# vandenheuvel/rust-lp

Hardware: AMD Instinct MI355X
Metric: simplex iterations/sec (higher is better)
Workload: dtype f64; 1 GPU; dense10k: synthetic dense LP 10000x10000 f64 (+10000 slack columns), SteepestDescent, dense tableau with blocked f64-MFMA updates; m=10000, n=10000, seed=20250002, engine=tableau, update_block=64, parallelism=single GPU, solves=1

## Files before the change

include/relp_engine.h:

```cpp
#ifndef RELP_ENGINE_H
#define RELP_ENGINE_H

#include <stdint.h>

#ifdef __cplusplus
extern "C" {
#endif

typedef struct relp_engine relp_engine_t;

typedef enum {
    RELP_OK = 0,
    RELP_E_ARG = -1,
    RELP_E_HIP = -2,
    RELP_E_ZERO_PIVOT = -3,
    RELP_E_SINGULAR = -4,
    RELP_E_STATE = -5,
    RELP_E_UNSUPPORTED = -6,
    RELP_E_ALLOC = -7
} relp_status_t;

typedef enum {
    RELP_RUNNING = 0,
    RELP_OPTIMAL = 1,
// ... 134 lines not shown
                                  const double *rhs, relp_cutpool_t **pool);
relp_status_t relp_cutpool_destroy(relp_engine_t *h, relp_cutpool_t *pool);
relp_status_t relp_cutpool_set_active(relp_engine_t *h, relp_cutpool_t *pool, const int32_t *ids, int32_t count, int32_t flag);
relp_status_t relp_cutpool_slacks(relp_engine_t *h, relp_cutpool_t *pool, double *out_count);
relp_status_t relp_cutpool_separate(relp_engine_t *h, relp_cutpool_t *pool, int32_t segments, double tol, int32_t by_efficacy,
                                    int32_t *ids_out , double *slack_out , int32_t *found);
relp_status_t relp_cutpool_add(relp_engine_t *h, relp_cutpool_t *pool, const int32_t *ids, int32_t count);
relp_status_t relp_cutpool_stats(const relp_engine_t *h, const relp_cutpool_t *pool, int64_t *out4);
relp_status_t relp_from_basis(relp_engine_t *h, const int32_t *basis_columns_m);
relp_status_t relp_set_reinversion_interval(relp_engine_t *h, int64_t pivots);
int64_t       relp_reinversions(const relp_engine_t *h);
relp_status_t relp_flush(relp_engine_t *h);
relp_status_t relp_tab_flush_stats(relp_engine_t *h, int64_t *out2);
relp_status_t relp_retab_stats(const relp_engine_t *h, int64_t *out4);
int32_t       relp_tab_load_batch(const relp_engine_t *h);
int32_t       relp_update_block(const relp_engine_t *h);
relp_status_t relp_lu_stats(const relp_engine_t *h, int64_t *out8);
relp_status_t relp_lu_lookahead_stats(const relp_engine_t *h, int64_t *out4);
relp_status_t relp_lu_kernel_layout(const relp_engine_t *h, int32_t *out4);
relp_status_t relp_lu_set_device_factorisation(relp_engine_t *h, int32_t on);
relp_status_t relp_lu_device_factorisation_stats(const relp_engine_t *h, int64_t *out6);
relp_status_t relp_lu_factor_residual(relp_engine_t *h, double *out);

relp_status_t relp_lu_phase_cycles(relp_engine_t *h, int64_t *out16);

relp_status_t relp_basis_inverse_row(relp_engine_t *h, int32_t row, double *out_m);
relp_status_t relp_should_refactor(relp_engine_t *h, int32_t *out);
relp_status_t relp_generate_column_of(relp_engine_t *h, const int32_t *row_idx, const double *values, int32_t nnz, double *out_m);
relp_status_t relp_cost_difference_of(relp_engine_t *h, const int32_t *row_idx, const double *values, int32_t nnz, double *out);
relp_status_t relp_lu_change_basis(relp_engine_t *h, int32_t pivot_row_index);
// ... 71 lines not shown
```

rust-lp_amd/csrc/relp_abi.cpp:

```cpp
#include <cstring>
#include <new>

#include "relp_engine.hpp"

using relp::Engine;

struct relp_engine { Engine impl; };

#define H(h) ((h)->impl)

extern "C" {

void relp_default_config(relp_config_t* cfg) {
    std::memset(cfg, 0, sizeof(*cfg));
    cfg->device = -1;
    cfg->phase_one_rule = RELP_RULE_FIRST_PROFITABLE_WITH_MEMORY;
    cfg->phase_two_rule = RELP_RULE_STEEPEST_DESCENT;
    cfg->tol_cost = 1e-7; cfg->tol_pivot = 1e-5; cfg->tol_zero = 1e-11; cfg->tol_tie = 1e-9; cfg->tol_feas = 1e-7;
    cfg->poll_interval = 64;
    cfg->trace_capacity = 0;
    cfg->shard_rank = 0; cfg->shard_count = 1;
    cfg->update_block = -1;
    cfg->engine = RELP_ENGINE_REVISED;
}
// ... 132 lines not shown
                                    double* slack_out, int32_t* found) {
    return h ? H(h).cutpool_separate(pool, segments, tol, by_efficacy, ids_out, slack_out, found) : RELP_E_ARG;
}
relp_status_t relp_cutpool_add(relp_engine_t* h, relp_cutpool_t* pool, const int32_t* ids, int32_t count) { return h ? H(h).cutpool_add(pool, ids, count) : RELP_E_ARG; }
relp_status_t relp_cutpool_stats(const relp_engine_t* h, const relp_cutpool_t* pool, int64_t* out4) { return (h && out4) ? H(h).cutpool_stats(pool, out4) : RELP_E_ARG; }
relp_status_t relp_solve_relaxation(relp_engine_t* h, int64_t max_iters, int32_t* outcome) {
    return h ? H(h).solve_relaxation(max_iters, outcome) : RELP_E_ARG;
}
relp_status_t relp_from_basis(relp_engine_t* h, const int32_t* basis) { return (h && basis) ? H(h).from_basis(basis) : RELP_E_ARG; }

relp_status_t relp_flush(relp_engine_t* h) { return h ? H(h).flush() : RELP_E_ARG; }
relp_status_t relp_set_reinversion_interval(relp_engine_t* h, int64_t pivots) { return h ? H(h).set_reinversion_interval(pivots) : RELP_E_ARG; }
int64_t relp_reinversions(const relp_engine_t* h) { return h ? H(h).reinversions() : -1; }
int32_t relp_update_block(const relp_engine_t* h) { return h ? H(h).update_block() : -1; }
int32_t relp_tab_load_batch(const relp_engine_t* h) { return h ? H(h).tab_load_batch_size() : -1; }
relp_status_t relp_lu_stats(const relp_engine_t* h, int64_t* out8) { return (h && out8) ? H(h).lu_stats(out8) : RELP_E_ARG; }
relp_status_t relp_lu_lookahead_stats(const relp_engine_t* h, int64_t* out4) { return (h && out4) ? H(h).lu_lookahead_stats(out4) : RELP_E_ARG; }
relp_status_t relp_lu_kernel_layout(const relp_engine_t* h, int32_t* out4) { return (h && out4) ? H(h).lu_kernel_layout(out4) : RELP_E_ARG; }
relp_status_t relp_lu_set_device_factorisation(relp_engine_t* h, int32_t on) { return h ? H(h).lu_set_device_factorisation(on != 0) : RELP_E_ARG; }
relp_status_t relp_lu_factor_residual(relp_engine_t* h, double* out) { return (h && out) ? H(h).lu_factor_residual(out) : RELP_E_ARG; }
relp_status_t relp_lu_device_factorisation_stats(const relp_engine_t* h, int64_t* out6) { return (h && out6) ? H(h).luf_stats(out6) : RELP_E_ARG; }
relp_status_t relp_shard_inject_failure(relp_engine_t* h, int64_t after_pivots) { if (!h) return RELP_E_ARG; H(h).shard_inject_failure(after_pivots); return RELP_OK; }
relp_status_t relp_lu_phase_cycles(relp_engine_t* h, int64_t* out16) { return (h && out16) ? H(h).lu_phase_cycles(out16) : RELP_E_ARG; }
relp_status_t relp_basis_inverse_row(relp_engine_t* h, int32_t row, double* out_m) { return (h && out_m) ? H(h).basis_inverse_row(row, out_m) : RELP_E_ARG; }
relp_status_t relp_should_refactor(relp_engine_t* h, int32_t* out) { return (h && out) ? H(h).should_refactor(out) : RELP_E_ARG; }
relp_status_t relp_generate_column_of(relp_engine_t* h, const int32_t* idx, const double* val, int32_t nnz, double* out_m) {
    return h ? H(h).generate_column_of(idx, val, nnz, out_m) : RELP_E_ARG;
}
relp_status_t relp_cost_difference_of(relp_engine_t* h, const int32_t* idx, const double* val, int32_t nnz, double* out) {
    return h ? H(h).cost_difference_of(idx, val, nnz, out) : RELP_E_ARG;
// ... 101 lines not shown
```

rust-lp_amd/csrc/relp_engine.cpp:

```cpp
#include "relp_engine_internal.hpp"
#include "relp_gomory.hpp"

#include <algorithm>
#include <chrono>
#include <cmath>
#include <cstdio>
#include <cstdlib>
#include <cstring>
#include <limits>

namespace relp {

bool Engine::hip_ok(hipError_t e, const char* what) {
    if (e == hipSuccess) return true;
    err_ = std::string(what) + ": " + hipGetErrorString(e);
    return false;
}

Engine::~Engine() { rccl_release(); luf_release(); }

ColumnTable Engine::table() const {
    ColumnTable ct;
    ct.nr_artificial = lay_.nr_artificial;
    ct.nr_normal = lay_.nr_normal;
// ... 55 lines not shown
    stream_ = s;
    owns_stream_ = false;
    return RELP_OK;
}

Switches Switches::read() {
    Switches s;
    auto given = [](const char* name) { return std::getenv(name) != nullptr; };
    auto num = [](const char* name, int unset) { const char* e = std::getenv(name); return e ? std::atoi(e) : unset; };
    s.debug = given("RELP_DEBUG");
    s.pivot_guard_set = given("RELP_PIVOT_GUARD");
    if (s.pivot_guard_set) s.pivot_guard = std::atof(std::getenv("RELP_PIVOT_GUARD"));
    s.tab_flush_all = num("RELP_TAB_FLUSH_ALL", 0) != 0;
    s.tab_load_batch = num("RELP_TAB_LOAD_BATCH", 0);
    s.tab_w_split = num("RELP_TAB_W_SPLIT", 0);
    s.fused_update = num("RELP_FUSED_UPDATE", 1) != 0;
    s.lu_lookahead_set = given("RELP_LU_LOOKAHEAD");
    s.lu_lookahead = num("RELP_LU_LOOKAHEAD", 8);
    s.fuse_lanes = num("RELP_FUSE_LANES", 256);
    s.lu_device_factor = num("RELP_LU_DEVICE_FACTOR", 0);
    s.lu_pipeline_short = num("RELP_LU_PIPELINE_SHORT", 0) != 0;
    s.ft_big = num("RELP_FT_BIG", -1);
    s.ft_hyper_set = given("RELP_FT_HYPER");
    s.ft_hyper = num("RELP_FT_HYPER", 0x9);
    s.ft_grid_price = given("RELP_FT_GRID_PRICE") ? (num("RELP_FT_GRID_PRICE", 0) != 0 ? 1 : 0) : -1;
    if (given("RELP_LUF_BUMP_CAP")) s.luf_bump_cap = std::max(16, num("RELP_LUF_BUMP_CAP", 0));
    s.luf_dense = std::max(0, std::min(64, num("RELP_LUF_DENSE", 64)));
    s.luf_lds = num("RELP_LUF_LDS", 1) != 0;
    s.lu_peel_stacks = num("RELP_LU_PEEL_STACKS", 0) != 0;
    s.dump_basis_set = given("RELP_DUMP_BASIS");
// ... 115 lines not shown
        HIP_TRY(dT0_.alloc(ld_t_ * n_owned));
        HIP_TRY(dR0_.alloc(ld_r_ * (block_ + 1)));
        {
            flush_all_ = sw_.tab_flush_all;
            HIP_TRY(d_fstats_.alloc(2));
            if (!flush_all_) {
                HIP_TRY(d_fcols_.alloc(n_owned));
                HIP_TRY(d_fcount_.alloc(1));
                HIP_TRY(d_fmask_.alloc((n_owned + 63) / 64));
                HIP_TRY(d_R0c_.alloc(ld_r_ * block_));
            }
        }
        {
            load_batch_ = tab_load_batch(sw_.tab_load_batch);
            w_split_ = sw_.tab_w_split >= 1 ? std::min(sw_.tab_w_split, 16) : kTabSplitDefault;
        }
        {
            fused_update_ = sw_.fused_update;
            if (cfg_.pivot_rescue && cfg_.shard_count == 1) fused_update_ = false;
            if (fused_update_) {
                HIP_TRY(d_b_alt_.alloc(ld_b_));
                HIP_TRY(d_basis_alt_.alloc(lay_.m));
                HIP_TRY(d_shadow_.alloc(std::max(block_, 1) + 1));
                HIP_TRY(d_shadow_meta_.alloc_raw(2 * sizeof(int32_t)));
                const int32_t none[2] = {-1, 0};
                HIP_TRY(d_shadow_meta_.upload(none, 2, stream_));
            }
        }
        HIP_TRY(d_cost_store_.alloc(n_store_));
        HIP_TRY(d_idcol_.alloc(lay_.m));
// ... 113 lines not shown

void Engine::enqueue_price(int cost_mode, const double* vec, const PivotRecord* rec, int32_t p_lo, int32_t p_hi) {
    const ColumnTable ct = table();
    if (lu_) {
        launch_price_csc(csc(), ct, vec, d_d_, 0, lay_.nr_normal, cost_mode, SelectPartials{}, rec, stream_);
        launch_price_virtual(ct, vec, d_d_, cost_mode, rec, stream_);
        return;
    }
    launch_price_structural(A_base(), ld_a_, ct, vec, d_d_, p_lo, p_hi, cost_mode, rec, stream_);
    if (p_lo > 0 || p_hi < lay_.nr_normal) launch_price_mask_unowned(ct, d_d_, p_lo, p_hi, rec, stream_);
    launch_price_virtual(ct, vec, d_d_, cost_mode, rec, stream_);
}

void Engine::enqueue_iteration_tableau(int rule) {
    const TableauView tv = tview();
    const DeferredUpdate du = deferred();
    const SelectPartials sp = tab_partials(rule);
    if (fused_update_ && in_loop_) {
        prof_begin(RELP_K_FTRAN);
        launch_tab_select_column_rmin(tv, du, sp, tab_scan_blocks(lay_.sc_hi - lay_.sc_lo), d_alpha_, d_b_, tolerances(), d_rmin_,
                                      d_rec_, stream_, d_shadow_, d_shadow_meta_);
        prof_end();
        prof_begin(RELP_K_PRICE);
        launch_tab_ratio_update_all(tv, du, sp, lay_.m, d_alpha_, d_b_, d_b_alt_, d_basis_, d_basis_alt_, d_in_basis_, d_trace_,
                                    trace_cap_, tolerances(), d_rmin_, d_shadow_, d_shadow_meta_, d_rec_, stream_);
        prof_end();
        d_b_.swap(d_b_alt_);
        d_basis_.swap(d_basis_alt_);
        shadow_pending_ = true;
        if (++since_flush_ >= block_) enqueue_flush();
        return;
    }
    tab_settle();
// ... 1878 lines not shown
```

rust-lp_amd/csrc/relp_engine.hpp:

```cpp
#pragma once
#include <hip/hip_runtime.h>

#include <cstdint>
#include <chrono>
#include <condition_variable>
#include <functional>
#include <memory>
#include <mutex>
#include <string>
#include <thread>
#include <vector>

#include "../../include/relp_engine.h"
#include "relp_buffers.hpp"
#include "relp_kernels.h"
#include "relp_layout.hpp"
#include "relp_cutpool.hpp"
#include "relp_lu.hpp"
#include "relp_pack.hpp"

namespace relp {
struct DevicePool {
    PoolImage image;
    DeviceBuf<int64_t> d_slice_ptr;
// ... 41 lines not shown
    ~HostPool() {
        for (Slot& s : slot) {
            if (!s.th.joinable()) continue;
            { std::lock_guard<std::mutex> lk(s.mu); s.stop = true; }
            s.cv.notify_all();
            s.th.join();
        }
    }
};

struct Switches {
    bool debug = false;
    bool pivot_guard_set = false; double pivot_guard = 0.0;
    bool tab_flush_all = false;
    int tab_load_batch = 0, tab_w_split = 0;
    bool fused_update = true;
    bool lu_lookahead_set = false; int lu_lookahead = 8;
    int fuse_lanes = 256;
    int lu_device_factor = 0;
    bool lu_pipeline_short = false;
    int ft_big = -1;
    bool ft_hyper_set = false; int ft_hyper = 0x9;
    int ft_grid_price = -1;
    int luf_bump_cap = INT32_MAX;
    int luf_dense = 64;
    bool luf_lds = true;
    bool lu_peel_stacks = false;
    bool dump_basis_set = false; std::string dump_basis;
    bool retab_global = false;
    int retab_groups = 0;
// ... 120 lines not shown

    int32_t nr_rows() const { return lay_.m; }
    int32_t nr_columns() const { return lay_.nr_columns(); }
    int32_t phase() const { return phase_; }
    int32_t nr_artificial() const { return lay_.nr_artificial; }
    relp_status_t get_objective(double* out);
    relp_status_t get_vector(int which, double* out);
    relp_status_t get_basis_indices(int32_t* out);
    relp_status_t get_basis_inverse(double* out);
    relp_status_t current_bfs(int32_t* cols, double* vals, int32_t cap, int32_t* count);
    relp_status_t get_iterations(int64_t* out);
    relp_status_t get_degenerate_pivots(int64_t* out);
    relp_status_t tab_flush_stats(int64_t* out2);
    relp_status_t retab_stats(int64_t* out4) const;
    int32_t tab_load_batch_size() const { return tableau_ ? load_batch_ : 0; }
    relp_status_t get_trace(int32_t* phase, int32_t* entering, int32_t* row, int32_t* leaving, int64_t cap,
                            int64_t* count);
    relp_status_t check_basis(double* max_identity_error, double* max_basic_cost, double* min_b);

    relp_status_t profile_enable(bool enable, int64_t max_launches, int32_t sample_every);
    relp_status_t profile_read(int kernel_id, int64_t* launches, double* total_ms);

    void shard_ranges(int32_t* col_lo, int32_t* col_hi, int32_t* row_lo, int32_t* row_hi, int32_t* stride) const;
    int64_t candidate_len() const { return lay_.candidate_len; }
    int64_t rho_len() const { return ld_b_; }
    relp_status_t shard_price(double* dev_candidate);
    relp_status_t shard_select_column(const double* dev_candidates, int32_t count);
    relp_status_t shard_ftran(double* dev_alpha_slice);
    relp_status_t shard_ratio(const double* dev_alpha_slices, int32_t count, double* dev_rho);
    relp_status_t shard_update(const double* dev_rho);
// ... 24 lines not shown
    int64_t since_flush_ = 0;
    DeviceBuf<double> d_v_;
    DeviceBuf<double> d_W_, d_wr_, d_R_;
    DeviceBuf<int32_t> d_S_, d_pos_of_row_;
    DeviceBuf<double> d_part_k1_;
    DeviceBuf<int32_t> d_part_j_;
    bool tableau_ = false;
    DeviceBuf<double> dT0_; int64_t ld_t_ = 0;
    DeviceBuf<double> dR0_; int64_t ld_r_ = 0;
    bool flush_all_ = false;
    DeviceBuf<int32_t> d_fcols_, d_fcount_;
    DeviceBuf<unsigned long long> d_fmask_, d_fstats_;
    DeviceBuf<double> d_R0c_;
    FlushList flush_list() const;
    int32_t load_batch_ = 0, w_split_ = 0;
    DeviceBuf<double> d_cost_store_;
    DeviceBuf<int32_t> d_idcol_;
    bool fused_update_ = false, shadow_pending_ = false;
    DeviceBuf<double> d_b_alt_, d_shadow_;
    DeviceBuf<int32_t> d_basis_alt_, d_shadow_meta_;
    DeviceBuf<double> d_rmin_;
    int32_t n_store_ = 0;
    int32_t tab_na_ = 0;
    bool tab_partials_valid_ = false;
    static constexpr int kRepriceEveryFlushes = 8;
    int32_t flushes_since_reprice_ = 0;
    std::vector<int32_t> idcol_h_;
    std::vector<double> cost_store_h_;
    bool in_loop_ = false;
    void tab_settle();
// ... 273 lines not shown
```

rust-lp_amd/csrc/relp_kernels.h:

```cpp
#pragma once
#include <hip/hip_runtime.h>
#include <stdint.h>

#include "relp_layout.hpp"
#include "relp_pool.hpp"
#include "relp_trial.hpp"

namespace relp {

enum DeviceOutcome : int32_t { DEV_RUNNING = 0, DEV_NO_CANDIDATE = 1, DEV_NO_ROW = 2 };

struct PivotRecord {
    int32_t outcome;
    int32_t q;
    double  d_q;
    int32_t r;
    int32_t leaving;
    double  alpha_r;
    double  b_r;
    double  minus_objective;
    long long iterations;
    int32_t last_selected;
    int32_t phase;
    int32_t owner_has_row;
// ... 5 lines not shown
    int32_t degenerate;
    int32_t p_now;
    int32_t pad2_;
};

struct DeferredUpdate {
    double*  W;
    int64_t  ld;
    int32_t  kmax;
    int32_t* S;
    int32_t* pos_of_row;
    double*  wr;
    double*  R;
    int32_t  batch;
    int32_t  w_split;
};

struct ColumnTable {
    int32_t nr_artificial;
    int32_t nr_normal;
    int32_t nr_virtual;
    int32_t nr_constraints;
    const int32_t* column_to_row;
    const int32_t* bound_row;
    const int32_t* vrow0;
    const int32_t* vrow1;
    const int32_t* vsign;
    const double*  cost;
    int32_t cut_row0 = 0;
    int32_t nr_cuts = 0;
// ... 253 lines not shown
void launch_tab_update_all(const TableauView& tv, const DeferredUpdate& du, SelectPartials sp, int32_t m,
                           const double* alpha, double* b, int32_t* basis_indices, uint8_t* in_basis, int32_t* trace,
                           int64_t trace_cap, PivotRecord* rec, hipStream_t s);
struct FlushList {
    int32_t*            cols;
    int32_t*            count;
    unsigned long long* mask;
    double*             R0c;
    int64_t             ld;
    unsigned long long* stats;
};
static constexpr int32_t kTabLoadBatchDefault = 8;
static constexpr int32_t kTabSplitDefault = 2;
static constexpr int32_t kTabSplitCUs = 256;
int32_t tab_load_batch(int32_t wanted);
void launch_tab_flush(const TableauView& tv, const DeferredUpdate& du, const PivotRecord* rec, const FlushList& fl,
                      hipStream_t s);
void launch_tab_ratio_update_all(const TableauView& tv, const DeferredUpdate& du, SelectPartials sp, int32_t m,
                                 const double* alpha, const double* b_in, double* b_out, const int32_t* basis_in,
                                 int32_t* basis_out, uint8_t* in_basis, int32_t* trace, int64_t trace_cap, Tolerances tol,
                                 const double* rmin, double* shadow, int32_t* shadow_meta, PivotRecord* rec, hipStream_t s,
                                 const double* msgs = nullptr, int32_t count = 0, int64_t msg_len = 0, int32_t rule = 0);
void launch_tab_apply_shadow(const DeferredUpdate& du, double* shadow, int32_t* shadow_meta, hipStream_t s);
void launch_tab_gather_columns(const TableauView& tv, const int32_t* cols, double* out, hipStream_t s);
void launch_tab_row(const TableauView& tv, const DeferredUpdate& du, int32_t row, double* out, const PivotRecord* rec,
                    hipStream_t s);
void launch_dual_bmin(const double* b, int32_t m, double tol_feas, double* bmin, const PivotRecord* rec, hipStream_t s);
void launch_dual_select_row(const double* b, const int32_t* basis_indices, int32_t m, double tol_feas, double tol_tie,
                            const double* bmin, PivotRecord* rec, hipStream_t s);
void launch_dual_row(const TableauView& tv, const DeferredUpdate& du, SelectPartials sp, const double* b,
// ... 126 lines not shown
```

rust-lp_amd/csrc/relp_kernels_tableau.hip:

```cpp
#include "relp_device_common.h"
#include <type_traits>

namespace relp {

typedef double double4_t __attribute__((ext_vector_type(4)));

template <int B, class Use>
__device__ __forceinline__ void for_pending(const double* base, int64_t stride, int64_t x, int n, Use&& use) {
    int j0 = 0;
    for (; j0 + B <= n; j0 += B) {
        double v[B];
#pragma unroll
        for (int t = 0; t < B; ++t) v[t] = base[(int64_t)(j0 + t) * stride + x];
#pragma unroll
        for (int t = 0; t < B; ++t) use(j0 + t, v[t]);
    }
    if (B > 1 && j0 < n) {
        double v[B];
#pragma unroll
        for (int t = 0; t < B; ++t) v[t] = j0 + t < n ? base[(int64_t)(j0 + t) * stride + x] : 0.0;
#pragma unroll
        for (int t = 0; t < B; ++t)
            if (j0 + t < n) use(j0 + t, v[t]);
    }
// ... 243 lines not shown
    }
}

template <int B>
__global__ __launch_bounds__(kThreads) void k_tab_update_all(TableauView tv, DeferredUpdate du, SelectPartials sp,
                                                             int nb_row, int m, const double* __restrict__ alpha,
                                                             double* __restrict__ b, int32_t* __restrict__ basis_indices,
                                                             uint8_t* __restrict__ in_basis, int32_t* __restrict__ trace,
                                                             int64_t trace_cap, PivotRecord* rec) {
    const PivotRecord R = *rec;
    if (R.outcome != DEV_RUNNING) return;
    if ((int)blockIdx.x < nb_row) tab_row_update_body<B>(tv, du, sp, R, blockIdx.x);
    else tab_update_w_vectors_body<B>(du, m, alpha, b, basis_indices, in_basis, trace, trace_cap, R, rec, blockIdx.x - nb_row);
}

template <int B>
__global__ __launch_bounds__(kThreads) void k_tab_ratio_update_all(TableauView tv, DeferredUpdate du, SelectPartials sp, int nb_row,
                                                                   int m, const double* alpha,
                                                                   const double* __restrict__ b_in, double* __restrict__ b_out,
                                                                   const int32_t* __restrict__ basis_in,
                                                                   int32_t* __restrict__ basis_out, uint8_t* in_basis,
                                                                   int32_t* __restrict__ trace, int64_t trace_cap, Tolerances tol,
                                                                   const double* rmin, int nblk,
                                                                   double* __restrict__ shadow, int32_t* __restrict__ shadow_meta,
                                                                   PivotRecord* rec, const double* __restrict__ msgs, int count,
                                                                   int64_t msg_len, int rule, int split) {
    const double first = (!msgs && (int)threadIdx.x < nblk) ? rmin[threadIdx.x] : INFINITY;
    PivotRecord R = *rec;
    const bool w_half = (int)blockIdx.x >= nb_row;
    const int part = w_half ? ((int)blockIdx.x - nb_row) / nblk : 0;
    const int wblock = (int)blockIdx.x - nb_row - part * nblk;
    const int i = wblock * kThreads + threadIdx.x;
    const bool lead = w_half && part == 0;
    const bool mine = lead && i < m;
    if (R.outcome != DEV_RUNNING) {
        if (mine) { b_out[i] = b_in[i]; basis_out[i] = basis_in[i]; }
        return;
    }
    if (msgs) {
        int q_win = 0;
        double d_win = 0.0;
        const int win = candidate_winner_staged(msgs, count, msg_len, rule, tol.tie, &q_win, &d_win);
        if (win < 0) {
            if (mine) { b_out[i] = b_in[i]; basis_out[i] = basis_in[i]; }
            if (lead && wblock == 0 && threadIdx.x == 0) record_candidate(rec, rule, -1, 0, 0.0);
            return;
        }
        R.q = q_win;
        R.d_q = d_win;
        if (rule == 1) R.last_selected = R.q;
        alpha = msgs + win * msg_len + 3;
        rmin = alpha + m;
    }
    int r, leaving;
    ratio_blocks_pick<kThreads>(alpha, b_in, basis_in, m, tol, rmin, nblk, &r, &leaving, first, !msgs);
    if (r < 0) {
        if (mine) { b_out[i] = b_in[i]; basis_out[i] = basis_in[i]; }
        if (lead && wblock == 0 && threadIdx.x == 0) rec->outcome = DEV_NO_ROW;
        return;
    }
    __shared__ double s_wr[kMaxEta];
    __shared__ double s_ab[2];
    __shared__ int s_jt;
    const int p_old = R.p_now;
    stage_w_row(du, r, p_old, s_wr);
    if (threadIdx.x == 0) {
        s_ab[0] = alpha[r]; s_ab[1] = b_in[r];
        const int slot = du.pos_of_row[r];
        s_jt = slot < 0 ? p_old : slot;
    }
// ... 40 lines not shown
        rec->r = r; rec->leaving = leaving; rec->alpha_r = alpha_r; rec->b_r = b_r;
        rec->n_eta_old = p_old; rec->eta_target = jt;
        if (jt >= p_old) { du.S[p_old] = r; du.pos_of_row[r] = p_old; rec->n_eta = p_old + 1; }
        pivot_bookkeeping(R.phase, R.iterations, R.minus_objective, R.d_q, br, q, r, leaving, in_basis, trace, trace_cap, rec);
    }
}

__global__ void k_tab_apply_shadow(DeferredUpdate du, double* __restrict__ shadow, int32_t* __restrict__ shadow_meta) {
    const int row = shadow_meta[0], len = shadow_meta[1];
    if (row < 0) return;
    for (int j = threadIdx.x; j < len; j += blockDim.x) du.W[(int64_t)j * du.ld + row] = shadow[j];
    __syncthreads();
    if (threadIdx.x == 0) shadow_meta[0] = -1;
}

template <int B>
__global__ __launch_bounds__(kThreads) void k_tab_select_column(TableauView tv, DeferredUpdate du, SelectPartials sp,
                                                                int count, double* alpha, double* msg,
                                                                const double* b, Tolerances tol,
                                                                double* rmin, PivotRecord* rec,
                                                                const double* shadow, int32_t* shadow_meta) {
    const int outcome = rec->outcome, p = rec->n_eta;
    if (shadow_meta) {
        const int srow = shadow_meta[0], slen = shadow_meta[1];
        if (srow >= 0 && srow / kThreads == (int)blockIdx.x) {
            if ((int)threadIdx.x < slen) du.W[(int64_t)threadIdx.x * du.ld + srow] = shadow[threadIdx.x];
            __syncthreads();
            if (threadIdx.x == 0) shadow_meta[0] = -1;
        }
        if (blockIdx.x == 0 && threadIdx.x == 0) rec->p_now = p;
    }
    double k1 = INFINITY;
    int bj = 0x7fffffff;
    if ((int)threadIdx.x < count) { k1 = sp.k1[threadIdx.x]; bj = sp.j[threadIdx.x]; }
    const int i = blockIdx.x * kThreads + threadIdx.x;
    const double b_i = (rmin && i < tv.m) ? b[i] : 0.0;
    if (outcome != DEV_RUNNING) return;
    __shared__ double s_vs[kMaxEta];
    tab_select_entering<kThreads>(tv, sp, count, k1, bj);
    if (bj == 0x7fffffff) {
        if (msg) {
            if (i < tv.m) alpha[i] = 0.0;
            if (i == 0) { msg[0] = INFINITY; msg[1] = 0.0; msg[2] = 0.0; }
        } else if (blockIdx.x == 0 && threadIdx.x == 0) {
            rec->outcome = DEV_NO_CANDIDATE;
            if (sp.rule == 1) rec->last_selected = -1;
        }
        return;
    }
    const int cq = bj + tv.col_off;
    if (blockIdx.x == 0 && threadIdx.x == 0) {
        if (msg) { msg[0] = k1; msg[1] = (double)bj; msg[2] = tv.d[cq]; }
        else {
            rec->q = bj;
            rec->d_q = tv.d[cq];
            rec->key1 = k1;
            if (sp.rule == 1) rec->last_selected = bj;
        }
    }
    if ((int)threadIdx.x < p) s_vs[threadIdx.x] = tv.R0[(int64_t)threadIdx.x * tv.ld_r + cq];
    const double t0 = i < tv.m ? tv.T0[(int64_t)cq * tv.ld_t + i] : 0.0;
    __syncthreads();
    double ratio = INFINITY;
    if (i < tv.m) {
        const double a = tab_column_entry<B>(du, i, p, s_vs, t0);
        alpha[i] = a;
        const double bz = b_i <= tol.zero ? 0.0 : b_i;
        if (a > tol.pivot) ratio = bz / a;
    }
    if (!rmin) return;
    ratio = block_min_value<kThreads>(ratio);
    if (threadIdx.x == 0) rmin[blockIdx.x] = ratio;
}

__global__ __launch_bounds__(kSingleBlock) void k_ratio_blocks(const double* __restrict__ alpha, const double* __restrict__ b,
                                                               const int32_t* __restrict__ basis_indices, int m,
                                                               Tolerances tol, DeferredUpdate du,
                                                               const double* __restrict__ rmin, int nblk, PivotRecord* rec) {
    const int outcome = rec->outcome, p = rec->n_eta;
    const double first = (int)threadIdx.x < nblk ? rmin[threadIdx.x] : INFINITY;
    if (outcome != DEV_RUNNING) return;
    ratio_blocks_body<kSingleBlock>(alpha, b, basis_indices, m, tol, du, rmin, nblk, p, rec, first, true);
}
// ... 1039 lines not shown
    if (blockIdx.x == 0 && threadIdx.x < kTrialUnit) {
        for (int s = 0; s < t.count; ++s) {
            const int64_t bytes = t.seg[s].bytes, whole = bytes / kTrialUnit * kTrialUnit;
            if (whole + (int64_t)threadIdx.x < bytes)
                static_cast<uint8_t*>(t.seg[s].dst)[whole + threadIdx.x] = static_cast<const uint8_t*>(t.seg[s].src)[whole + threadIdx.x];
        }
    }
}

int32_t tab_scan_blocks(int32_t n_owned_columns) { return cdiv(n_owned_columns, kThreads); }

int32_t tab_load_batch(int32_t wanted) {
    return (wanted == 1 || wanted == 8 || wanted == 16 || wanted == 32) ? wanted : kTabLoadBatchDefault;
}

template <class Launch>
static void with_load_batch(int32_t batch, Launch&& launch) {
    switch (tab_load_batch(batch)) {
    case 1:  launch(std::integral_constant<int, 1>{}); break;
    case 16: launch(std::integral_constant<int, 16>{}); break;
    case 32: launch(std::integral_constant<int, 32>{}); break;
    default: launch(std::integral_constant<int, 8>{}); break;
    }
    static_assert(kTabLoadBatchDefault == 8, "the default of tab_load_batch is the switch's default case");
}

void launch_tab_build(const TableauView& tv, const double* A, int64_t ld_a, const ColumnTable& ct, hipStream_t s) {
    const int64_t total = (int64_t)tv.m * (tv.c_hi - tv.c_lo);
    if (total <= 0) return;
    hipLaunchKernelGGL(k_tab_build, dim3(element_blocks(total)), dim3(256), 0, s, tv, A, ld_a, ct);
// ... 33 lines not shown
    with_load_batch(du.batch, [&](auto B) {
        hipLaunchKernelGGL((k_tab_row_update<decltype(B)::value>), dim3(tab_scan_blocks(tv.c_hi - tv.c_lo)), dim3(kThreads), 0, s, tv, du, sp,
                           rec);
    });
}

void launch_tab_update_vectors(int32_t m, const double* alpha, double* b, int32_t* basis_indices, uint8_t* in_basis,
                               int32_t* trace, int64_t trace_cap, PivotRecord* rec, hipStream_t s) {
    hipLaunchKernelGGL(k_tab_update_vectors, dim3(cdiv(m, 256)), dim3(256), 0, s, m, alpha, b, basis_indices, in_basis,
                       trace, trace_cap, rec);
}

void launch_tab_select_column_rmin(const TableauView& tv, const DeferredUpdate& du, SelectPartials sp, int32_t count,
                                   double* alpha, const double* b, Tolerances tol, double* rmin, PivotRecord* rec,
                                   hipStream_t s, const double* shadow, int32_t* shadow_meta) {
    with_load_batch(du.batch, [&](auto B) {
        hipLaunchKernelGGL((k_tab_select_column<decltype(B)::value>), dim3(cdiv(tv.m, kThreads)), dim3(kThreads), 0, s, tv, du, sp, count, alpha,
                           (double*)nullptr, b, tol, rmin, rec, shadow, shadow_meta);
    });
}

void launch_tab_ratio_update_all(const TableauView& tv, const DeferredUpdate& du, SelectPartials sp, int32_t m,
                                 const double* alpha, const double* b_in, double* b_out, const int32_t* basis_in,
                                 int32_t* basis_out, uint8_t* in_basis, int32_t* trace, int64_t trace_cap, Tolerances tol,
                                 const double* rmin, double* shadow, int32_t* shadow_meta, PivotRecord* rec, hipStream_t s,
                                 const double* msgs, int32_t count, int64_t msg_len, int32_t rule) {
    const int nb_row = tv.c_hi > tv.c_lo ? tab_scan_blocks(tv.c_hi - tv.c_lo) : 0;
    const int nb_w = cdiv(m, kThreads);
    int split = tab_load_batch(du.batch) == 1 ? 1 : std::max(1, std::min({(int)du.w_split, (int)du.kmax, (kTabSplitCUs - nb_row) / nb_w}));
    with_load_batch(du.batch, [&](auto B) {
        hipLaunchKernelGGL((k_tab_ratio_update_all<decltype(B)::value>), dim3(nb_row + split * nb_w), dim3(kThreads), 0, s, tv, du, sp, nb_row, m,
                           alpha, b_in, b_out, basis_in, basis_out, in_basis, trace, trace_cap, tol, rmin, nb_w, shadow,
                           shadow_meta, rec, msgs, (int)count, msg_len, (int)rule, split);
    });
}

void launch_tab_apply_shadow(const DeferredUpdate& du, double* shadow, int32_t* shadow_meta, hipStream_t s) {
    hipLaunchKernelGGL(k_tab_apply_shadow, dim3(1), dim3(128), 0, s, du, shadow, shadow_meta);
}

void launch_ratio_blocks(const double* alpha, const double* b, const int32_t* basis_indices, int32_t m, Tolerances tol,
                         const DeferredUpdate& du, const double* rmin, PivotRecord* rec, hipStream_t s) {
    hipLaunchKernelGGL(k_ratio_blocks, dim3(1), dim3(kSingleBlock), 0, s, alpha, b, basis_indices, m, tol, du, rmin,
                       cdiv(m, kThreads), rec);
}

void launch_tab_select_column_msg(const TableauView& tv, const DeferredUpdate& du, SelectPartials sp, int32_t count,
                                  double* msg, const double* b, Tolerances tol, PivotRecord* rec, hipStream_t s,
                                  const double* shadow, int32_t* shadow_meta) {
    with_load_batch(du.batch, [&](auto B) {
        hipLaunchKernelGGL((k_tab_select_column<decltype(B)::value>), dim3(cdiv(tv.m, kThreads)), dim3(kThreads), 0, s, tv, du, sp, count, msg + 3,
                           msg, b, tol, msg + 3 + tv.m, rec, shadow, shadow_meta);
    });
}

void launch_tab_select_candidate_ratio(const double* msgs, int32_t count, int64_t msg_len, int32_t m, double* alpha,
                                       const double* b, const int32_t* basis_indices, int32_t rule, Tolerances tol,
                                       const DeferredUpdate& du, int32_t forced_row, PivotRecord* rec, hipStream_t s) {
    hipLaunchKernelGGL(k_tab_select_candidate_ratio, dim3(1), dim3(kSingleBlock), 0, s, msgs, count, msg_len, m, alpha, b,
                       basis_indices, rule, tol, du, forced_row, rec);
}

void launch_tab_zero_level_scan(const TableauView& tv, const DeferredUpdate& du, SelectPartials sp, int32_t row,
                                int32_t nr_artificial, Tolerances tol, const PivotRecord* rec, hipStream_t s) {
    if (tv.c_hi <= tv.c_lo) return;
    with_load_batch(du.batch, [&](auto B) {
// ... 559 lines not shown
```

rust-lp_amd/engine.py:

```python
from __future__ import annotations

import ctypes as C
import os
from typing import List, Optional, Tuple

import numpy as np

from .matrix_data import MatrixData

_HERE = os.path.dirname(os.path.abspath(__file__))
LIB_PATH = os.path.join(_HERE, "librelp_engine.so")

FIRST_PROFITABLE, FIRST_PROFITABLE_WITH_MEMORY, STEEPEST_DESCENT = 0, 1, 2
RUNNING, OPTIMAL, UNBOUNDED, INFEASIBLE, PHASE_ONE_DONE, NO_ROW_PHASE_ONE = range(6)
GOMORY_FRACTIONAL, GOMORY_MIXED = 0, 1
GOMORY_CUT, GOMORY_NOT_INTEGER, GOMORY_FRACTION, GOMORY_ARTIFICIAL, GOMORY_CONTINUOUS = range(5)
BRANCH_EVALUATED, BRANCH_NOT_STRUCTURAL, BRANCH_FRACTION = range(3)
OUTCOME_NAMES = {RUNNING: "running", OPTIMAL: "optimal", UNBOUNDED: "unbounded", INFEASIBLE: "infeasible",
                 PHASE_ONE_DONE: "phase_one_done", NO_ROW_PHASE_ONE: "no_row_phase_one"}
(K_PRICE, K_SELECT_COLUMN, K_BUILD_COLUMN, K_FTRAN, K_RATIO, K_UPDATE_VECTORS, K_UPDATE_INVERSE, K_APPLY_W,
 K_UPDATE_W, K_FLUSH, K_FT_RUN) = range(11)
KERNEL_NAMES = ["price", "select_column", "build_column", "ftran", "ratio", "update_vectors", "update_inverse",
                "apply_w", "update_w", "flush", "ft_run"]
ENGINE_REVISED, ENGINE_TABLEAU, ENGINE_LU, ENGINE_AUTO = 0, 1, 2, 3
# ... 86 lines not shown
    "relp_pool_add": (C.c_int, [C.c_void_p, C.c_void_p, C.c_void_p, C.c_int32]),
    "relp_pool_stats": (C.c_int, [C.c_void_p, C.c_void_p, C.POINTER(C.c_int64)]),
    "relp_cutpool_create": (C.c_int, [C.c_void_p, C.c_int32, C.c_void_p, C.c_void_p, C.c_void_p, C.c_void_p, C.POINTER(C.c_void_p)]),
    "relp_cutpool_destroy": (C.c_int, [C.c_void_p, C.c_void_p]),
    "relp_cutpool_set_active": (C.c_int, [C.c_void_p, C.c_void_p, C.c_void_p, C.c_int32, C.c_int32]),
    "relp_cutpool_slacks": (C.c_int, [C.c_void_p, C.c_void_p, C.c_void_p]),
    "relp_cutpool_separate": (C.c_int, [C.c_void_p, C.c_void_p, C.c_int32, C.c_double, C.c_int32, C.c_void_p, C.c_void_p,
                                        C.POINTER(C.c_int32)]),
    "relp_cutpool_add": (C.c_int, [C.c_void_p, C.c_void_p, C.c_void_p, C.c_int32]),
    "relp_cutpool_stats": (C.c_int, [C.c_void_p, C.c_void_p, C.POINTER(C.c_int64)]),
    "relp_solve_relaxation": (C.c_int, [C.c_void_p, C.c_int64, C.POINTER(C.c_int32)]),
    "relp_from_basis": (C.c_int, [C.c_void_p, C.c_void_p]),
    "relp_flush": (C.c_int, [C.c_void_p]),
    "relp_update_block": (C.c_int32, [C.c_void_p]),
    "relp_tab_load_batch": (C.c_int32, [C.c_void_p]),
    "relp_tab_flush_stats": (C.c_int, [C.c_void_p, C.POINTER(C.c_int64)]),
    "relp_retab_stats": (C.c_int, [C.c_void_p, C.POINTER(C.c_int64)]),
    "relp_lu_stats": (C.c_int, [C.c_void_p, C.POINTER(C.c_int64)]),
    "relp_lu_lookahead_stats": (C.c_int, [C.c_void_p, C.POINTER(C.c_int64)]),
    "relp_lu_kernel_layout": (C.c_int, [C.c_void_p, C.POINTER(C.c_int32)]),
    "relp_lu_set_device_factorisation": (C.c_int, [C.c_void_p, C.c_int32]),
    "relp_lu_device_factorisation_stats": (C.c_int, [C.c_void_p, C.POINTER(C.c_int64)]),
    "relp_lu_factor_residual": (C.c_int, [C.c_void_p, C.POINTER(C.c_double)]),
    "relp_lu_phase_cycles": (C.c_int, [C.c_void_p, C.POINTER(C.c_int64)]),
    "relp_basis_inverse_row": (C.c_int, [C.c_void_p, C.c_int32, C.c_void_p]),
    "relp_should_refactor": (C.c_int, [C.c_void_p, C.POINTER(C.c_int32)]),
    "relp_generate_column_of": (C.c_int, [C.c_void_p, C.c_void_p, C.c_void_p, C.c_int32, C.c_void_p]),
    "relp_cost_difference_of": (C.c_int, [C.c_void_p, C.c_void_p, C.c_void_p, C.c_int32, C.POINTER(C.c_double)]),
    "relp_lu_change_basis": (C.c_int, [C.c_void_p, C.c_int32]),
    "relp_lu_set_factors": (C.c_int, [C.c_void_p] + [C.c_void_p] * 6),
# ... 493 lines not shown

    def solve_relaxation(self, max_iters: int = 1 << 40) -> int:
        oc = C.c_int32()
        self._ck(self._lib.relp_solve_relaxation(self._h, max_iters, C.byref(oc)))
        return oc.value

    def flush(self) -> None:
        self._ck(self._lib.relp_flush(self._h))

    def update_block(self) -> int:
        return self._lib.relp_update_block(self._h)

    def load_batch(self) -> int:
        return self._lib.relp_tab_load_batch(self._h)

    def flush_stats(self) -> Tuple[int, int]:
        out = (C.c_int64 * 2)()
        self._ck(self._lib.relp_tab_flush_stats(self._h, out))
        return int(out[0]), int(out[1])

    def retab_stats(self) -> Tuple[int, int, int, int]:
        out = (C.c_int64 * 4)()
        self._ck(self._lib.relp_retab_stats(self._h, out))
        return tuple(int(v) for v in out)

    def engine_kind(self) -> int:
        return int(self._lib.relp_engine_kind(self._h))

    def robust_stats(self) -> dict:
        out = (C.c_int64 * 4)()
# ... 436 lines not shown
```

Before: 45010 iterations/s.

## Split tableau column generation across wavefront slices per row block

The column-selection kernel can now give each block 64 or 128 rows instead of 256, splitting the pending eta updates across wavefront slices that accumulate through shared memory. With m=10000 this launches more blocks, and the deferred W reads are spread over more CUs. The ratio/update kernel is made aware of the new row-block count. The serial shared-memory chaining across slices adds syncs and register arrays, and whether the default path picks smaller rows depends on m versus kTabSplitCUs.

```diff
diff --git a/include/relp_engine.h b/include/relp_engine.h
--- a/include/relp_engine.h
+++ b/include/relp_engine.h
@@ -172,6 +172,8 @@
 relp_status_t relp_tab_flush_stats(relp_engine_t *h, int64_t *out2);
 relp_status_t relp_retab_stats(const relp_engine_t *h, int64_t *out4);
 int32_t       relp_tab_load_batch(const relp_engine_t *h);
+int32_t       relp_tab_column_rows(const relp_engine_t *h);
+int32_t       relp_tab_column_rows_for(int32_t wanted, int32_t m);
 int32_t       relp_update_block(const relp_engine_t *h);
 relp_status_t relp_lu_stats(const relp_engine_t *h, int64_t *out8);
 relp_status_t relp_lu_lookahead_stats(const relp_engine_t *h, int64_t *out4);
diff --git a/rust-lp_amd/csrc/relp_abi.cpp b/rust-lp_amd/csrc/relp_abi.cpp
--- a/rust-lp_amd/csrc/relp_abi.cpp
+++ b/rust-lp_amd/csrc/relp_abi.cpp
@@ -170,6 +170,8 @@
 int64_t relp_reinversions(const relp_engine_t* h) { return h ? H(h).reinversions() : -1; }
 int32_t relp_update_block(const relp_engine_t* h) { return h ? H(h).update_block() : -1; }
 int32_t relp_tab_load_batch(const relp_engine_t* h) { return h ? H(h).tab_load_batch_size() : -1; }
+int32_t relp_tab_column_rows(const relp_engine_t* h) { return h ? H(h).tab_column_rows_size() : -1; }
+int32_t relp_tab_column_rows_for(int32_t wanted, int32_t m) { return relp::tab_column_rows(wanted, m); }
 relp_status_t relp_lu_stats(const relp_engine_t* h, int64_t* out8) { return (h && out8) ? H(h).lu_stats(out8) : RELP_E_ARG; }
 relp_status_t relp_lu_lookahead_stats(const relp_engine_t* h, int64_t* out4) { return (h && out4) ? H(h).lu_lookahead_stats(out4) : RELP_E_ARG; }
 relp_status_t relp_lu_kernel_layout(const relp_engine_t* h, int32_t* out4) { return (h && out4) ? H(h).lu_kernel_layout(out4) : RELP_E_ARG; }
diff --git a/rust-lp_amd/csrc/relp_engine.cpp b/rust-lp_amd/csrc/relp_engine.cpp
--- a/rust-lp_amd/csrc/relp_engine.cpp
+++ b/rust-lp_amd/csrc/relp_engine.cpp
@@ -93,6 +93,7 @@
     s.tab_flush_all = num("RELP_TAB_FLUSH_ALL", 0) != 0;
     s.tab_load_batch = num("RELP_TAB_LOAD_BATCH", 0);
     s.tab_w_split = num("RELP_TAB_W_SPLIT", 0);
+    s.tab_column_rows = num("RELP_TAB_COLUMN_ROWS", 0);
     s.fused_update = num("RELP_FUSED_UPDATE", 1) != 0;
     s.lu_lookahead_set = given("RELP_LU_LOOKAHEAD");
     s.lu_lookahead = num("RELP_LU_LOOKAHEAD", 8);
@@ -238,6 +239,7 @@
         {
             load_batch_ = tab_load_batch(sw_.tab_load_batch);
             w_split_ = sw_.tab_w_split >= 1 ? std::min(sw_.tab_w_split, 16) : kTabSplitDefault;
+            col_rows_wanted_ = sw_.tab_column_rows;
         }
         {
             fused_update_ = sw_.fused_update;
@@ -381,9 +383,10 @@
 
 void Engine::enqueue_iteration_tableau(int rule) {
     const TableauView tv = tview();
-    const DeferredUpdate du = deferred();
+    DeferredUpdate du = deferred();
     const SelectPartials sp = tab_partials(rule);
     if (fused_update_ && in_loop_) {
+        du.col_rows = tab_column_rows_size();
         prof_begin(RELP_K_FTRAN);
         launch_tab_select_column_rmin(tv, du, sp, tab_scan_blocks(lay_.sc_hi - lay_.sc_lo), d_alpha_, d_b_, tolerances(), d_rmin_,
                                       d_rec_, stream_, d_shadow_, d_shadow_meta_);
diff --git a/rust-lp_amd/csrc/relp_engine.hpp b/rust-lp_amd/csrc/relp_engine.hpp
--- a/rust-lp_amd/csrc/relp_engine.hpp
+++ b/rust-lp_amd/csrc/relp_engine.hpp
@@ -79,6 +79,7 @@
     bool pivot_guard_set = false; double pivot_guard = 0.0;
     bool tab_flush_all = false;
     int tab_load_batch = 0, tab_w_split = 0;
+    int tab_column_rows = 0;
     bool fused_update = true;
     bool lu_lookahead_set = false; int lu_lookahead = 8;
     int fuse_lanes = 256;
@@ -229,6 +230,11 @@
     relp_status_t tab_flush_stats(int64_t* out2);
     relp_status_t retab_stats(int64_t* out4) const;
     int32_t tab_load_batch_size() const { return tableau_ ? load_batch_ : 0; }
+    int32_t tab_column_rows_size() const {
+        if (!tableau_) return 0;
+        const bool asked = col_rows_wanted_ == 64 || col_rows_wanted_ == 128 || col_rows_wanted_ == 256;
+        return !asked && block_ > 64 ? 256 : tab_column_rows(col_rows_wanted_, lay_.m);
+    }
     relp_status_t get_trace(int32_t* phase, int32_t* entering, int32_t* row, int32_t* leaving, int64_t cap,
                             int64_t* count);
     relp_status_t check_basis(double* max_identity_error, double* max_basic_cost, double* min_b);
@@ -283,6 +289,7 @@
     DeviceBuf<double> d_R0c_;
     FlushList flush_list() const;
     int32_t load_batch_ = 0, w_split_ = 0;
+    int32_t col_rows_wanted_ = 0;
     DeviceBuf<double> d_cost_store_;
     DeviceBuf<int32_t> d_idcol_;
     bool fused_update_ = false, shadow_pending_ = false;
diff --git a/rust-lp_amd/csrc/relp_kernels.h b/rust-lp_amd/csrc/relp_kernels.h
--- a/rust-lp_amd/csrc/relp_kernels.h
+++ b/rust-lp_amd/csrc/relp_kernels.h
@@ -43,6 +43,7 @@
     double*  R;
     int32_t  batch;
     int32_t  w_split;
+    int32_t  col_rows = 0;
 };
 
 struct ColumnTable {
@@ -326,6 +327,7 @@
 static constexpr int32_t kTabSplitDefault = 2;
 static constexpr int32_t kTabSplitCUs = 256;
 int32_t tab_load_batch(int32_t wanted);
+int32_t tab_column_rows(int32_t wanted, int32_t m);
 void launch_tab_flush(const TableauView& tv, const DeferredUpdate& du, const PivotRecord* rec, const FlushList& fl,
                       hipStream_t s);
 void launch_tab_ratio_update_all(const TableauView& tv, const DeferredUpdate& du, SelectPartials sp, int32_t m,
diff --git a/rust-lp_amd/csrc/relp_kernels_tableau.hip b/rust-lp_amd/csrc/relp_kernels_tableau.hip
--- a/rust-lp_amd/csrc/relp_kernels_tableau.hip
+++ b/rust-lp_amd/csrc/relp_kernels_tableau.hip
@@ -281,22 +281,23 @@
     else tab_update_w_vectors_body<B>(du, m, alpha, b, basis_indices, in_basis, trace, trace_cap, R, rec, blockIdx.x - nb_row);
 }
 
-template <int B>
+template <int B, int RPB>
 __global__ __launch_bounds__(kThreads) void k_tab_ratio_update_all(TableauView tv, DeferredUpdate du, SelectPartials sp, int nb_row,
                                                                    int m, const double* alpha,
                                                                    const double* __restrict__ b_in, double* __restrict__ b_out,
                                                                    const int32_t* __restrict__ basis_in,
                                                                    int32_t* __restrict__ basis_out, uint8_t* in_basis,
                                                                    int32_t* __restrict__ trace, int64_t trace_cap, Tolerances tol,
-                                                                   const double* rmin, int nblk,
+                                                                   const double* rmin, int nblk, int nb_w_other,
                                                                    double* __restrict__ shadow, int32_t* __restrict__ shadow_meta,
                                                                    PivotRecord* rec, const double* __restrict__ msgs, int count,
                                                                    int64_t msg_len, int rule, int split) {
     const double first = (!msgs && (int)threadIdx.x < nblk) ? rmin[threadIdx.x] : INFINITY;
     PivotRecord R = *rec;
     const bool w_half = (int)blockIdx.x >= nb_row;
-    const int part = w_half ? ((int)blockIdx.x - nb_row) / nblk : 0;
-    const int wblock = (int)blockIdx.x - nb_row - part * nblk;
+    const int nb_w = RPB == kThreads ? nblk : nb_w_other;
+    const int part = w_half ? ((int)blockIdx.x - nb_row) / nb_w : 0;
+    const int wblock = (int)blockIdx.x - nb_row - part * nb_w;
     const int i = wblock * kThreads + threadIdx.x;
     const bool lead = w_half && part == 0;
     const bool mine = lead && i < m;
@@ -320,7 +321,7 @@
         rmin = alpha + m;
     }
     int r, leaving;
-    ratio_blocks_pick<kThreads>(alpha, b_in, basis_in, m, tol, rmin, nblk, &r, &leaving, first, !msgs);
+    ratio_blocks_pick<kThreads>(alpha, b_in, basis_in, m, tol, rmin, nblk, &r, &leaving, first, !msgs, RPB);
     if (r < 0) {
         if (mine) { b_out[i] = b_in[i]; basis_out[i] = basis_in[i]; }
         if (lead && wblock == 0 && threadIdx.x == 0) rec->outcome = DEV_NO_ROW;
@@ -391,16 +392,18 @@
     if (threadIdx.x == 0) shadow_meta[0] = -1;
 }
 
-template <int B>
+template <int B, int R, int NW>
 __global__ __launch_bounds__(kThreads) void k_tab_select_column(TableauView tv, DeferredUpdate du, SelectPartials sp,
                                                                 int count, double* alpha, double* msg,
                                                                 const double* b, Tolerances tol,
                                                                 double* rmin, PivotRecord* rec,
                                                                 const double* shadow, int32_t* shadow_meta) {
+    static_assert(R == 64 || R == 128 || R == kThreads, "whole wavefronts per slice");
+    constexpr int S = kThreads / R;
     const int outcome = rec->outcome, p = rec->n_eta;
     if (shadow_meta) {
         const int srow = shadow_meta[0], slen = shadow_meta[1];
-        if (srow >= 0 && srow / kThreads == (int)blockIdx.x) {
+        if (srow >= 0 && srow / R == (int)blockIdx.x) {
             if ((int)threadIdx.x < slen) du.W[(int64_t)threadIdx.x * du.ld + srow] = shadow[threadIdx.x];
             __syncthreads();
             if (threadIdx.x == 0) shadow_meta[0] = -1;
@@ -410,8 +413,9 @@
     double k1 = INFINITY;
     int bj = 0x7fffffff;
     if ((int)threadIdx.x < count) { k1 = sp.k1[threadIdx.x]; bj = sp.j[threadIdx.x]; }
-    const int i = blockIdx.x * kThreads + threadIdx.x;
-    const double b_i = (rmin && i < tv.m) ? b[i] : 0.0;
+    const int slice = R == kThreads ? 0 : (int)threadIdx.x / R;
+    const int i = blockIdx.x * R + (R == kThreads ? (int)threadIdx.x : (int)threadIdx.x % R);
+    const double b_i = (rmin && i < tv.m && slice == S - 1) ? b[i] : 0.0;
     if (outcome != DEV_RUNNING) return;
     __shared__ double s_vs[kMaxEta];
     tab_select_entering<kThreads>(tv, sp, count, k1, bj);
@@ -435,15 +439,49 @@
             if (sp.rule == 1) rec->last_selected = bj;
         }
     }
-    if ((int)threadIdx.x < p) s_vs[threadIdx.x] = tv.R0[(int64_t)threadIdx.x * tv.ld_r + cq];
-    const double t0 = i < tv.m ? tv.T0[(int64_t)cq * tv.ld_t + i] : 0.0;
-    __syncthreads();
     double ratio = INFINITY;
-    if (i < tv.m) {
-        const double a = tab_column_entry<B>(du, i, p, s_vs, t0);
-        alpha[i] = a;
-        const double bz = b_i <= tol.zero ? 0.0 : b_i;
-        if (a > tol.pivot) ratio = bz / a;
+    if constexpr (R == kThreads) {
+        if ((int)threadIdx.x < p) s_vs[threadIdx.x] = tv.R0[(int64_t)threadIdx.x * tv.ld_r + cq];
+        const double t0 = i < tv.m ? tv.T0[(int64_t)cq * tv.ld_t + i] : 0.0;
+        __syncthreads();
+        if (i < tv.m) {
+            const double a = tab_column_entry<B>(du, i, p, s_vs, t0);
+            alpha[i] = a;
+            const double bz = b_i <= tol.zero ? 0.0 : b_i;
+            if (a > tol.pivot) ratio = bz / a;
+        }
+    } else {
+        const double vq = (int)threadIdx.x < p ? tv.R0[(int64_t)threadIdx.x * tv.ld_r + cq] : 0.0;
+        double a = (i < tv.m && slice == 0) ? tv.T0[(int64_t)cq * tv.ld_t + i] : 0.0;
+        const int share = (p + S - 1) / S;
+        const int j_lo = min(slice * share, p);
+        const int cnt = i < tv.m ? min(share, p - j_lo) : 0;
+        const double* col = du.W + (int64_t)j_lo * du.ld + i;
+        double w[NW];
+#pragma unroll
+        for (int t = 0; t < NW; ++t) w[t] = t < cnt ? col[(int64_t)t * du.ld] : 0.0;
+        if ((int)threadIdx.x < p) s_vs[threadIdx.x] = vq;
+        __syncthreads();
+        double v[NW];
+#pragma unroll
+        for (int t = 0; t < NW; ++t) v[t] = s_vs[min(j_lo + t, kMaxEta - 1)];
+        __shared__ double s_acc[R];
+        const int x = (int)threadIdx.x % R;
+#pragma unroll
+        for (int s = 0; s < S; ++s) {
+            if (s > 0) __syncthreads();
+            if (slice == s) {
+                if (s > 0) a = s_acc[x];
+#pragma unroll
+                for (int t = 0; t < NW; ++t) a = t < cnt ? fma(w[t], v[t], a) : a;
+                if (s < S - 1) s_acc[x] = a;
+            }
+        }
+        if (slice == S - 1 && i < tv.m) {
+            alpha[i] = a;
+            const double bz = b_i <= tol.zero ? 0.0 : b_i;
+            if (a > tol.pivot) ratio = bz / a;
+        }
     }
     if (!rmin) return;
     ratio = block_min_value<kThreads>(ratio);
@@ -1513,6 +1551,15 @@
     return (wanted == 1 || wanted == 8 || wanted == 16 || wanted == 32) ? wanted : kTabLoadBatchDefault;
 }
 
+int32_t tab_column_rows(int32_t wanted, int32_t m) {
+    if (wanted == 64 || wanted == 128 || wanted == kThreads) return wanted;
+    for (int32_t rows : {64, 128})
+        if (cdiv(m, rows) <= kTabSplitCUs) return rows;
+    return kThreads;
+}
+
+static int column_rows_of(const DeferredUpdate& du) { return du.col_rows == 64 || du.col_rows == 128 ? du.col_rows : kThreads; }
+
 template <class Launch>
 static void with_load_batch(int32_t batch, Launch&& launch) {
     switch (tab_load_batch(batch)) {
@@ -1576,10 +1623,30 @@
 void launch_tab_select_column_rmin(const TableauView& tv, const DeferredUpdate& du, SelectPartials sp, int32_t count,
                                    double* alpha, const double* b, Tolerances tol, double* rmin, PivotRecord* rec,
                                    hipStream_t s, const double* shadow, int32_t* shadow_meta) {
-    with_load_batch(du.batch, [&](auto B) {
-        hipLaunchKernelGGL((k_tab_select_column<decltype(B)::value>), dim3(cdiv(tv.m, kThreads)), dim3(kThreads), 0, s, tv, du, sp, count, alpha,
-                           (double*)nullptr, b, tol, rmin, rec, shadow, shadow_meta);
-    });
+    const int rows = column_rows_of(du);
+    if (rows == kThreads) {
+        with_load_batch(du.batch, [&](auto B) {
+            hipLaunchKernelGGL((k_tab_select_column<decltype(B)::value, kThreads, 1>), dim3(cdiv(tv.m, kThreads)), dim3(kThreads), 0, s, tv, du, sp,
+                               count, alpha, (double*)nullptr, b, tol, rmin, rec, shadow, shadow_meta);
+        });
+        return;
+    }
+    const int need = cdiv(du.kmax, kThreads / rows);
+    static_assert(kMaxEta <= 2 * 64, "the largest array takes half of the pending rows");
+    auto launch = [&](auto R, auto NW) {
+        hipLaunchKernelGGL((k_tab_select_column<kTabLoadBatchDefault, decltype(R)::value, decltype(NW)::value>), dim3(cdiv(tv.m, rows)),
+                           dim3(kThreads), 0, s, tv, du, sp, count, alpha, (double*)nullptr, b, tol, rmin, rec, shadow, shadow_meta);
+    };
+    static_assert(kMaxEta <= 4 * 32, "32 registers take a quarter of the pending rows");
+    if (need <= 16) {
+        if (rows == 128) launch(std::integral_constant<int, 128>{}, std::integral_constant<int, 16>{});
+        else launch(std::integral_constant<int, 64>{}, std::integral_constant<int, 16>{});
+    } else if (need <= 32) {
+        if (rows == 128) launch(std::integral_constant<int, 128>{}, std::integral_constant<int, 32>{});
+        else launch(std::integral_constant<int, 64>{}, std::integral_constant<int, 32>{});
+    } else {
+        launch(std::integral_constant<int, 128>{}, std::integral_constant<int, 64>{});
+    }
 }
 
 void launch_tab_ratio_update_all(const TableauView& tv, const DeferredUpdate& du, SelectPartials sp, int32_t m,
@@ -1589,11 +1656,17 @@
                                  const double* msgs, int32_t count, int64_t msg_len, int32_t rule) {
     const int nb_row = tv.c_hi > tv.c_lo ? tab_scan_blocks(tv.c_hi - tv.c_lo) : 0;
     const int nb_w = cdiv(m, kThreads);
+    const int rpb = msgs ? kThreads : column_rows_of(du);
     int split = tab_load_batch(du.batch) == 1 ? 1 : std::max(1, std::min({(int)du.w_split, (int)du.kmax, (kTabSplitCUs - nb_row) / nb_w}));
+    auto launch = [&](auto B, auto RPB) {
+        hipLaunchKernelGGL((k_tab_ratio_update_all<decltype(B)::value, decltype(RPB)::value>), dim3(nb_row + split * nb_w), dim3(kThreads), 0, s,
+                           tv, du, sp, nb_row, m, alpha, b_in, b_out, basis_in, basis_out, in_basis, trace, trace_cap, tol, rmin,
+                           cdiv(m, rpb), nb_w, shadow, shadow_meta, rec, msgs, (int)count, msg_len, (int)rule, split);
+    };
     with_load_batch(du.batch, [&](auto B) {
-        hipLaunchKernelGGL((k_tab_ratio_update_all<decltype(B)::value>), dim3(nb_row + split * nb_w), dim3(kThreads), 0, s, tv, du, sp, nb_row, m,
-                           alpha, b_in, b_out, basis_in, basis_out, in_basis, trace, trace_cap, tol, rmin, nb_w, shadow,
-                           shadow_meta, rec, msgs, (int)count, msg_len, (int)rule, split);
+        if (rpb == 64) launch(B, std::integral_constant<int, 64>{});
+        else if (rpb == 128) launch(B, std::integral_constant<int, 128>{});
+        else launch(B, std::integral_constant<int, kThreads>{});
     });
 }
 
@@ -1611,7 +1684,7 @@
                                   double* msg, const double* b, Tolerances tol, PivotRecord* rec, hipStream_t s,
                                   const double* shadow, int32_t* shadow_meta) {
     with_load_batch(du.batch, [&](auto B) {
-        hipLaunchKernelGGL((k_tab_select_column<decltype(B)::value>), dim3(cdiv(tv.m, kThreads)), dim3(kThreads), 0, s, tv, du, sp, count, msg + 3,
+        hipLaunchKernelGGL((k_tab_select_column<decltype(B)::value, kThreads, 1>), dim3(cdiv(tv.m, kThreads)), dim3(kThreads), 0, s, tv, du, sp, count, msg + 3,
                            msg, b, tol, msg + 3 + tv.m, rec, shadow, shadow_meta);
     });
 }
diff --git a/rust-lp_amd/engine.py b/rust-lp_amd/engine.py
--- a/rust-lp_amd/engine.py
+++ b/rust-lp_amd/engine.py
@@ -124,6 +124,8 @@
     "relp_flush": (C.c_int, [C.c_void_p]),
     "relp_update_block": (C.c_int32, [C.c_void_p]),
     "relp_tab_load_batch": (C.c_int32, [C.c_void_p]),
+    "relp_tab_column_rows": (C.c_int32, [C.c_void_p]),
+    "relp_tab_column_rows_for": (C.c_int32, [C.c_int32, C.c_int32]),
     "relp_tab_flush_stats": (C.c_int, [C.c_void_p, C.POINTER(C.c_int64)]),
     "relp_retab_stats": (C.c_int, [C.c_void_p, C.POINTER(C.c_int64)]),
     "relp_lu_stats": (C.c_int, [C.c_void_p, C.POINTER(C.c_int64)]),
@@ -647,6 +649,9 @@
     def load_batch(self) -> int:
         return self._lib.relp_tab_load_batch(self._h)
 
+    def column_rows(self) -> int:
+        return self._lib.relp_tab_column_rows(self._h)
+
     def flush_stats(self) -> Tuple[int, int]:
         out = (C.c_int64 * 2)()
         self._ck(self._lib.relp_tab_flush_stats(self._h, out))
```

After: 46240 iterations/s (median of 6 runs). 1.03x the previous value.
